# OneWalkman/EDGE-YOLO

Measured on AMD Instinct MI355X. Metric: images/sec @ 640x640 fp16 (EdgeLine-YOLO detection forward path: backbone + DWT neck + GFLv2 head decode + batched NMS), higher is better.
Workload: dtype f16; 1 GPU; yolo11n-test.yaml (scale n, nc=80) predict path, 640x640, batch 32/GPU, conf 0.25 iou 0.7 max_det 300, random-init weights, default head biases (DENSE NMS regime: mean detections/img 300); regime=dense, global_batch=32, imgsz=640, nc=80

## Files before the change

### edge-yolo_amd/_lib.py

```python
import ctypes as C
import os

import torch

_HERE = os.path.dirname(os.path.abspath(__file__))
LIB_PATH = os.path.join(_HERE, "csrc", "libedgeyolo_hip.so")

F16, F32 = 0, 1
ACT_NONE, ACT_SILU, ACT_RELU, ACT_SIGMOID = 0, 1, 2, 3
ATTN_AREA_F32, ATTN_AREA_F16, ATTN_AREA_MFMA = 401, 402, 403
ATTN_FLASH_MFMA, ATTN_FLASH_F32, ATTN_FLASH_F16 = 500, 501, 502
DWG_PLAIN, DWG_GATE, DWG_RESIDUAL = 0, 1, 2
MASK_GT_STACK, MASK_GT_INDEX = 0, 1


class HipLibraryError(RuntimeError):
    pass


class ConvDesc(C.Structure):
    _fields_ = [
        ("dtype", C.c_int32), ("B", C.c_int32), ("H", C.c_int32), ("W", C.c_int32), ("Ho", C.c_int32), ("Wo", C.c_int32),
        ("Cout", C.c_int32), ("k", C.c_int32), ("stride", C.c_int32), ("pad", C.c_int32), ("act", C.c_int32), ("nsrc", C.c_int32),
        ("src", C.c_void_p * 2), ("src_C", C.c_int32 * 2), ("src_cstride", C.c_int32 * 2), ("src_up", C.c_int32 * 2),
        ("w", C.c_void_p), ("bias", C.c_void_p), ("y", C.c_void_p), ("y_cstride", C.c_int32),
        ("res", C.c_void_p), ("res_cstride", C.c_int32), ("out_scale", C.c_float),
        ("addz", C.c_void_p), ("addz_cstride", C.c_int32), ("addz_H", C.c_int32), ("addz_W", C.c_int32), ("ngroup", C.c_int32),
        ("src_gstride", C.c_int64), ("y_gstride", C.c_int64), ("w_gstride", C.c_int64), ("w_gmax", C.c_int32),
    ]


class ConvDirectDesc(C.Structure):
    _fields_ = [
        ("dtype", C.c_int32), ("B", C.c_int32), ("H", C.c_int32), ("W", C.c_int32), ("Cin", C.c_int32), ("Ho", C.c_int32),
        ("Wo", C.c_int32), ("Cout", C.c_int32), ("k", C.c_int32), ("stride", C.c_int32), ("pad", C.c_int32), ("groups", C.c_int32),
        ("act", C.c_int32), ("x", C.c_void_p), ("x_cstride", C.c_int32), ("w_oihw", C.c_void_p), ("bias", C.c_void_p),
        ("y", C.c_void_p), ("y_cstride", C.c_int32),
    ]


class BlockStage(C.Structure):
    _fields_ = [
        ("op", C.c_int32), ("H", C.c_int32), ("W", C.c_int32), ("Ho", C.c_int32), ("Wo", C.c_int32),
        ("k", C.c_int32), ("stride", C.c_int32), ("act", C.c_int32), ("nsrc", C.c_int32),
        ("src", C.c_int64 * 2), ("src_ext", C.c_int32 * 2), ("src_img", C.c_int64 * 2), ("src_cs", C.c_int32 * 2), ("src_C", C.c_int32 * 2),
        ("w", C.c_void_p), ("bias", C.c_void_p), ("w_g", C.c_int64), ("w_gmax", C.c_int32),
        ("y", C.c_int64), ("y_ext", C.c_int32), ("y_img", C.c_int64), ("y_cs", C.c_int32), ("Cout", C.c_int32),
        ("has_res", C.c_int32), ("res", C.c_int64), ("res_ext", C.c_int32), ("res_img", C.c_int64), ("res_cs", C.c_int32),
        ("has_addz", C.c_int32), ("addz", C.c_int64), ("addz_ext", C.c_int32), ("addz_img", C.c_int64), ("addz_cs", C.c_int32), ("addz_H", C.c_int32),
        ("addz_W", C.c_int32), ("out_scale", C.c_float),
        ("ngroup", C.c_int32), ("src_g", C.c_int64), ("y_g", C.c_int64), ("heads", C.c_int32),
        ("kpad", C.c_int32), ("nt_pack", C.c_int32), ("mt", C.c_int32), ("nti", C.c_int32), ("lds", C.c_int32), ("tile_nti", C.c_int32), ("tile_src_lds", C.c_int32 * 2), ("tile_src_lcs", C.c_int32 * 2), ("tile_y_lds", C.c_int32), ("tile_y_lcs", C.c_int32), ("tile_res_lds", C.c_int32), ("tile_res_lcs", C.c_int32), ("tile_lds_bytes", C.c_int32), ("zsy", C.c_float), ("zsx", C.c_float),
    ]
# ... 16 lines not shown
    "ey_conv_pack_nt": (_i, [_i]),
    "ey_conv_chain_klen": (_i, [_i]),
    "ey_conv_chain_kperm": (_i, [_i, _vp, _i]),
    "ey_conv_pw_chain": (_i, [_i, _i, _i, _i, _i, _i, _i, _vp, _i, _vp, _vp, _i, _vp, _vp, _i, _vp, _i, _vp]),
    "ey_conv2d_direct": (_i, [C.POINTER(ConvDirectDesc), _vp]),
    "ey_stem_conv": (_i, [_i, _i, _i, _i, _i, _i, _i, _i, _vp, _vp, _vp, _vp, _i, _vp]),
    "ey_dwconv": (_i, [_i, _i, _i, _i, _i, _i, _i, _vp, _i, _vp, _vp, _vp, _i, _vp]),
    "ey_dsconv": (_i, [_i, _i, _i, _i, _i, _i, _i, _i, _vp, _i, _vp, _vp, _i, _vp, _vp, _vp, _i, _vp, _i, _vp]),
    "ey_dsconv_toeplitz_bytes": (_sz, [_i, _i]),
    "ey_dsconv_pack_toeplitz": (_i, [_i, _i, _vp, _vp, _sz]),
    "ey_dsconv_tz": (_i, [_i, _i, _i, _i, _i, _i, _i, _i, _vp, _i, _vp, _vp, _vp, _i, _vp, _vp, _vp, _i, _vp, _i, _vp]),
    "ey_dsconv_last_variant": (_i, []),
    "ey_conv_pw_conv3s2": (_i, [_i, _i, _i, _i, _vp, _i, _i, _vp, _i, _i, _i, _vp, _vp, _i, _i, _vp, _vp, _i, _vp, _i, _vp]),
    "ey_stem_pair": (_i, [_i, _i, _i, _vp, _vp, _vp, _i, _i, _vp, _vp, _i, _vp, _i, _vp]),
    "ey_dsb_pair": (_i, [_i, _i, _i, _i, _i, _i, _i, _i, _vp, _i, _vp, _vp, _vp, _vp, _vp, _vp, _i, _vp, _i, _vp]),
    "ey_dwt_haar": (_i, [_i, _i, _i, _i, _i, _vp, _i, _vp, _i, _vp]),
    "ey_dwt": (_i, [_i, _i, _i, _i, _i, _i, _vp, _vp, _i, _vp, _i, _vp]),
    "ey_wavelet_z": (_i, [_i, _i, _i, _i, _i, _vp, _i, _vp, C.c_long, _vp, _vp, _vp, _i, _vp]),
    "ey_wavelet_z2": (_i, [_i, _i, _i, _i, _i, _i, _vp, _i, _vp, _vp, _i, _vp, C.c_long, _vp, _vp, _vp, _i, _vp]),
    "ey_sppf_pool": (_i, [_i, _i, _i, _i, _i, _vp, _i, _vp, _vp, _vp, _i, _vp]),
    "ey_copy_nhwc": (_i, [_i, _i, _i, _i, _i, _i, _vp, _i, _vp, _i, _vp]),
    "ey_scale_add_channels": (_i, [_i, _i, _i, _i, _i, _vp, _i, _vp, _vp, _i, _vp, _i, _vp]),
    "ey_avgpool2": (_i, [_i, _i, _i, _i, _i, _vp, _i, _vp, _i, _vp]),
    "ey_dwconv_s2": (_i, [_i, _i, _i, _i, _i, _i, _i, _vp, _i, _vp, _vp, _vp, _i, _vp]),
    "ey_hypergraph_workspace_bytes": (_sz, [_i, _i, _i, _i]),
    "ey_hypergraph_conv": (_i, [_i, _i, _i, _i, _i, _i, _i, _vp, _i, _vp, _i, _vp, _vp, _vp, _vp, _vp, _vp, _vp, _vp, _vp, _vp, _sz, _vp]),
    "ey_nchw_to_nhwc": (_i, [_i, _i, _i, _i, _i, _vp, _vp, _i, _vp]),
    "ey_nhwc_to_nchw": (_i, [_i, _i, _i, _i, _i, _vp, _i, _vp, _vp]),
    "ey_letterbox": (_i, [_i, _vp, _i, _i, _i, _vp, _i, _i, _i, _i, _i, _i, _i, _i, _vp]),
    "ey_copy_linear": (_i, [_vp, _vp, _sz, _vp]),
# ... 145 lines not shown
```

### edge-yolo_amd/csrc/api.cpp

```cpp
#include <stdarg.h>
#include <stdio.h>
#include <stddef.h>
#include <string.h>
#include "../../include/edgeyolo_hip.h"
#include "tune.h"

static thread_local char g_err[512] = "";

int ey_set_error(int code, const char* fmt, ...) {
  va_list ap;
  va_start(ap, fmt);
  vsnprintf(g_err, sizeof(g_err), fmt, ap);
  va_end(ap);
  return code;
}

extern "C" const char* ey_last_error(void) { return g_err; }
extern "C" int ey_version(void) { return 1; }
extern "C" size_t ey_abi_sizeof(int which) { return which == 0 ? sizeof(ey_conv_desc) : which == 1 ? sizeof(ey_conv_direct_desc) : 0; }

EyTune g_ey_tune;
#define EY_T(f) {#f, offsetof(EyTune, f)}
static const struct { const char* name; size_t off; } k_tunables[] = {
    EY_T(tiles_per_wave), EY_T(mt2_min_m), EY_T(small_m), EY_T(small_wmb), EY_T(halo_min_c), EY_T(ws_lds_kb), EY_T(ws_wg_cu), EY_T(ws_k3_minnt), EY_T(tile_wlds),
    EY_T(tile_s2_minc), EY_T(tile_s2_minm), EY_T(grid_div), EY_T(c3r), EY_T(tile_minwg), EY_T(tile_flat), EY_T(tile_mink), EY_T(pwr_m), EY_T(pwr_frags), EY_T(pw_m),
    EY_T(pw_waves), EY_T(pw_wmb), EY_T(ds_p), EY_T(tz_kmask), EY_T(tz_minpx), EY_T(ds_strip), EY_T(stem_mfma), EY_T(linattn_mfma), EY_T(softattn_mfma), EY_T(areaattn_mfma), EY_T(c3p), EY_T(c3p_min_m), EY_T(c3p_fast), EY_T(c3s), EY_T(c3s_mt4_m), EY_T(c3s_min_work), EY_T(c3s_cfg), EY_T(nms_fast_k), EY_T(nms_mask_wg), EY_T(sppf_min_wg), EY_T(sppf_cv), EY_T(dsb_pair), EY_T(dsb_max_px), EY_T(dsb_rb), EY_T(dsb_fixed), EY_T(dsb_p2), EY_T(stem_pair), EY_T(pw3), EY_T(pw3_min_px), EY_T(pw3_skew), EY_T(pwn), EY_T(pwn_max_m), EY_T(pwn_ntw), EY_T(pwc), EY_T(xcd_map), EY_T(nms_mask_k), EY_T(head_lean), EY_T(head_fuse)};
static long* tunable(const char* name) {
  if (!name) return nullptr;
  for (const auto& t : k_tunables)
    if (!strcmp(t.name, name)) return (long*)((char*)&g_ey_tune + t.off);
  return nullptr;
}
extern "C" int ey_tune_set(const char* name, long value) {
  long* p = tunable(name);
  if (!p) return ey_set_error(EY_EINVAL, "ey_tune_set: unknown tunable '%s'", name ? name : "(null)");
  *p = value;
  return EY_OK;
}
extern "C" long ey_tune_get(const char* name) {
  const long* p = tunable(name);
  return p ? *p : -1;
// ... 2 lines not shown
```

### edge-yolo_amd/csrc/dsb.hip

```cpp
#include "common.h"
#include "tune.h"

struct DsbP {
  int B, H, W, act, add;
  const void* x; int xCs; unsigned xBytes;
  const void* wdw1; const void* wpw1; const float* b1;
  const void* wdw2; const void* wpw2; const float* b2;
  void* y; int yCs;
  int RB, Kpad;
};

#define DSB_SLACK 8

template <int K, int KS, int P, bool LAST>
__device__ __forceinline__ void dsb_stage(const DsbP& p, int b, const f16* s_src, int srcW, int src_row0, const f16* s_w, const void* wpw, const float* bias_g,
                                          int row_lo, int row_hi, f16* s_dst, int dstW, int dst_row0, int dst_pad, const f16* s_res, int resW, int res_row0,
                                          int res_pad) {
  constexpr int C = 32 * KS, NT = 2 * KS, CP = C + 8, NX = P + K - 1;
  const int lane = threadIdx.x & 63, r = lane & 15, g = lane >> 4, wave = threadIdx.x >> 6, nwave = blockDim.x >> 6;
  const int ch0 = g * 4 * NT;
  Vec8<f16> af[KS][NT];
  {
    const __amdgpu_buffer_rsrc_t rw = ey_rsrc(wpw, (unsigned)(16 * NT * p.Kpad * (int)sizeof(f16)));
    const unsigned wvoff = (unsigned)((r * p.Kpad + 8 * g) * (int)sizeof(f16));
#pragma unroll
    for (int ks = 0; ks < KS; ++ks)
#pragma unroll
      for (int nt = 0; nt < NT; ++nt) BufLoad8<f16>::load(af[ks][nt], rw, wvoff, (nt * 16 * p.Kpad + ks * 32) * (int)sizeof(f16));
  }
  float bias[4 * NT];
#pragma unroll
  for (int i = 0; i < 4 * NT; ++i) bias[i] = bias_g ? bias_g[ch0 + i] : 0.f;
  const int WS = (p.W + P - 1) / P;
  const int nstrip = (row_hi - row_lo) * WS;
  for (int unit = wave; unit * 16 < nstrip; unit += nwave) {
    const int si = unit * 16 + r;
    const bool sv = si < nstrip;
    const int sic = sv ? si : nstrip - 1;
    const int ry = sic / WS, x0 = (sic - ry * WS) * P, oy = row_lo + ry;
    Vec8<f16> bf[KS][P];
#pragma unroll
    for (int ks = 0; ks < KS; ++ks) {
      const int cb = ks * 32 + 8 * g;
      float acc[P][8];
#pragma unroll
      for (int q = 0; q < P; ++q)
#pragma unroll
        for (int i = 0; i < 8; ++i) acc[q][i] = 0.f;
      const f16* base = s_src + ((oy - K / 2 - src_row0) * srcW + x0) * CP + cb;
#pragma unroll
      for (int ky = 0; ky < K; ++ky) {
        Vec8<f16> xr[NX];
#pragma unroll
        for (int j = 0; j < NX; ++j) xr[j].load(base + (ky * srcW + j) * CP);
#pragma unroll
        for (int kx = 0; kx < K; ++kx) {
          Vec8<f16> w;
          w.load(s_w + (ky * K + kx) * C + cb);
#pragma unroll
          for (int q = 0; q < P; ++q) ey_fma8_mix(xr[q + kx], w, acc[q]);
        }
      }
#pragma unroll
      for (int q = 0; q < P; ++q)
#pragma unroll
        for (int i = 0; i < 8; ++i) bf[ks][q].set(i, acc[q][i]);
    }
#pragma unroll
    for (int q = 0; q < P; ++q) {
      f32x4 pacc[NT];
#pragma unroll
      for (int nt = 0; nt < NT; ++nt) pacc[nt] = (f32x4)0.f;
#pragma unroll
      for (int ks = 0; ks < KS; ++ks)
#pragma unroll
        for (int nt = 0; nt < NT; ++nt) pacc[nt] = __builtin_amdgcn_mfma_f32_16x16x32_f16(af[ks][nt].v, bf[ks][q].v, pacc[nt], 0, 0, 0);
      const int ox = x0 + q;
      if (!sv || ox >= p.W) continue;
      float v[4 * NT];
#pragma unroll
      for (int nt = 0; nt < NT; ++nt)
// ... 19 lines not shown
            Vec8<f16> rr;
            rr.load(rp + 8 * h);
#pragma unroll
            for (int j = 0; j < 8; ++j) v[8 * h + j] += rr.get(j);
          }
          Vec8<f16> o;
#pragma unroll
          for (int j = 0; j < 8; ++j) o.set(j, v[8 * h + j]);
          o.store(yp + 8 * h);
        }
      }
    }
  }
}

template <int K1, int K2, int KS, int P1, int P2>
__global__ __launch_bounds__(512) void dsb_pair_kernel(DsbP p) {
  extern __shared__ __attribute__((aligned(16))) char smem[];
  constexpr int C = 32 * KS, CP = C + 8, CV = C / 8, R1 = K1 / 2, R2 = K2 / 2, PPI = 512 / CV;
  const int RI = p.RB + 2 * (R1 + R2), WI = p.W + 2 * R1, RM = p.RB + 2 * R2, WM = p.W + 2 * R2;
  f16* s_in = reinterpret_cast<f16*>(smem);
  f16* s_mid = s_in + (RI * WI + DSB_SLACK) * CP;
  f16* s_w1 = s_mid + (RM * WM + DSB_SLACK) * CP;
  f16* s_w2 = s_w1 + K1 * K1 * C;
  const int tid = threadIdx.x, b = blockIdx.y, y0 = blockIdx.x * p.RB;
  {
    const __amdgpu_buffer_rsrc_t rx = ey_rsrc(p.x, p.xBytes);
    const int cv = tid % CV, NP = RI * WI, iy0 = y0 - R1 - R2;
    constexpr int U = 4;
    int base = tid / CV;
    bool first = true;
    do {
// ... 19 lines not shown
          w.load((const f16*)p.wdw2 + v * 8);
          w.store(s_w2 + v * 8);
        }
      }
#pragma unroll
      for (int j = 0; j < U; ++j) {
        const int px = base + j * PPI;
        if (px < NP) t[j].store(s_in + px * CP + cv * 8);
      }
      base += U * PPI;
    } while (base < NP);
  }
  __syncthreads();
  {
    const int lo = y0 - R2 < 0 ? 0 : y0 - R2, hi = y0 + p.RB + R2 > p.H ? p.H : y0 + p.RB + R2;
    dsb_stage<K1, KS, P1, false>(p, b, s_in, WI, y0 - R1 - R2, s_w1, p.wpw1, p.b1, lo, hi, s_mid, WM, y0 - R2, R2, nullptr, 0, 0, 0);
  }
  __syncthreads();
  {
    const int hi = y0 + p.RB > p.H ? p.H : y0 + p.RB;
    dsb_stage<K2, KS, P2, true>(p, b, s_mid, WM, y0 - R2, s_w2, p.wpw2, p.b2, y0, hi, nullptr, 0, 0, 0, s_in, WI, y0 - R1 - R2, R1);
  }
}

static size_t dsb_lds_bytes(int W, int C, int k1, int k2, int RB) {
  const int CP = C + 8, r1 = k1 / 2, r2 = k2 / 2;
  return ((size_t)((RB + 2 * (r1 + r2)) * (W + 2 * r1) + DSB_SLACK) + (size_t)((RB + 2 * r2) * (W + 2 * r2) + DSB_SLACK)) * CP * 2 + (size_t)(k1 * k1 + k2 * k2) * C * 2;
}

static int dsb_band_rows(int B, int H, int W, int C, int k1, int k2) {
  static int ncu = 0;
  if (!ncu) {
    int dev = 0;
    hipDeviceProp_t prop;
    if (hipGetDevice(&dev) == hipSuccess && hipGetDeviceProperties(&prop, dev) == hipSuccess) ncu = prop.multiProcessorCount;
    if (ncu < 1) ncu = 256;
  }
// ... 49 lines not shown
  const int bands = (H + RB - 1) / RB;
  const size_t lds = dsb_lds_bytes(W, C, k1, k2, RB);
  hipStream_t st = (hipStream_t)stream;
  int P2 = (int)tune().dsb_p2;
  if (P2 != 1 && P2 != 2 && P2 != 4) P2 = RB * ((W + 1) / 2) < 64 ? 1 : 2;
#define DSB(KV, KSV)                                                          \
  if (k2 == KV && C == 32 * KSV) {                                            \
    if (P2 == 1) return dsb_launch<3, KV, KSV, 2, 1>(p, bands, lds, st);      \
    if (P2 == 4) return dsb_launch<3, KV, KSV, 2, 4>(p, bands, lds, st);      \
    return dsb_launch<3, KV, KSV, 2, 2>(p, bands, lds, st);                   \
  }
  DSB(5, 1) DSB(7, 1) DSB(5, 2) DSB(7, 2)
#undef DSB
  return ey_set_error(EY_EINVAL, "dsb_pair: k2=%d C=%d", k2, C);
}
```

### edge-yolo_amd/csrc/tune.h

```cpp
#pragma once
struct EyTune {
  long tiles_per_wave = 0;
  long mt2_min_m = 300000;
  long small_m = 100000;
  long small_wmb = 48;
  long halo_min_c = 48;
  long ws_lds_kb = 76;
  long ws_wg_cu = 2;
  long ws_k3_minnt = 0;
  long tile_wlds = 1;
  long tile_s2_minc = 64;
  long tile_s2_minm = 40000;
  long grid_div = 1;
  long c3p = 1;
  long c3p_min_m = 40000;
  long c3p_fast = 1;
  long c3s = 1;
  long c3s_mt4_m = 100000;
  long c3s_min_work = 20000;
  long c3s_cfg = 0;
  long c3r = 1;
  long tile_minwg = 400;
  long tile_flat = 1;
  long tile_mink = 0;
// ... 4 lines not shown
  long pw_wmb = 64;
  long xcd_map = 31;
  long pwc = 1;
  long pwn = 1;
  long pwn_max_m = 110000;
  long pwn_ntw = 0;
  long ds_p = 0;
  long tz_kmask = 168;
  long tz_minpx = 100000;
  long ds_strip = 1;
  long dsb_pair = 1;
  long dsb_max_px = 300000;
  long dsb_rb = 0;
  long dsb_p2 = 0;
  long dsb_fixed = 100;
  long stem_pair = 1;
  long pw3 = 1;
  long pw3_skew = 8;
  long pw3_min_px = 100000;
  long stem_mfma = 1;
  long linattn_mfma = 1;
  long softattn_mfma = 1;
  long areaattn_mfma = 1;
  long sppf_min_wg = 128;
  long sppf_cv = 0;
  long nms_mask_wg = 0;
  long nms_mask_k = 1536;
  long head_fuse = 2;
  long head_lean = 1;
  long nms_fast_k = 2048;
// ... 4 lines not shown
```

### edge-yolo_amd/nn/_ops.py

```python
import ctypes

import torch

from .. import _lib as L

TRACE = None
RECORD = None


def _no_block(what):
    if RECORD is not None:
        from ._block import BlockUnsupported
        raise BlockUnsupported(what)


class _NoTrace:
    def __enter__(self):
        return None

    def __exit__(self, *a):
        return False


_NT = _NoTrace()
# ... 448 lines not shown
        cs = L.cstride(x)
        if L.cstride(out) != cs or abs(((x.data_ptr() - base) // 2) % cs - ((out.data_ptr() - base) // 2) % cs) < c:
            return None
    wk1, _, wp1, b1, _, _ = _dsconv_pack(cv1, x, cv1._dw_folded, cv1._pw_folded, k1)
    wk2, _, wp2, b2, _, _ = _dsconv_pack(cv2, x, cv2._dw_folded, cv2._pw_folded, k2)
    try:
        with _tr(f"dsb_pair_kernel<{k1},{k2}>", _nb(x, out), 2.0 * B * H * W * c * (k1 * k1 + k2 * k2 + 2 * c), note=f"C{c} {H}x{W}{' +res' if add else ''}"):
            L.check(L.lib().ey_dsb_pair(L.dtype_code(x.dtype), B, H, W, c, k1, k2, L.ACT_SILU, x.data_ptr(), L.cstride(x), wk1.data_ptr(), wp1.data_ptr(),
                                        b1.data_ptr() if b1 is not None else None, wk2.data_ptr(), wp2.data_ptr(), b2.data_ptr() if b2 is not None else None,
                                        1 if add else 0, out.data_ptr(), L.cstride(out), L.stream()), "ey_dsb_pair")
    except NotImplementedError:
        return None
    return out


def dsconv(mod, x, dw_fn, pw_fn, k, act, out=None, res=None, dw_act=0):
    L.require_device(x, "dsconv")
    x = L.as_nhwc(x)
    B, c, H, W = x.shape
    es = x.element_size()
    if c % 8 or c > 256 or (L.cstride(x) * es) % 16 or x.data_ptr() % 16:
        return None

    wk, dwb, wp, bias, cout, tz = _dsconv_pack(mod, x, dw_fn, pw_fn, k)
    if out is None:
        out = L.empty_nhwc(B, cout, H, W, x.dtype, x.device)
    elif not L.is_nhwc_view(out) or tuple(out.shape) != (B, cout, H, W):
        raise ValueError("dsconv: out= must be an NHWC view of the output shape")
    if res is not None:
        res = L.as_nhwc(res)
# ... 786 lines not shown
```

### edge-yolo_amd/nn/modules/block.py

```python
import math

import torch
import torch.nn as nn
import torch.nn.functional as F

from .conv import Conv, DSConv, _Packed, fold_bn
from .. import _ops as ops
from ... import _lib as L

__all__ = ("DFL", "Proto", "SPPF", "C2f", "C3", "C3k", "C3k2", "Bottleneck", "Attention", "PSABlock", "C2PSA", "LinearAttention",
           "PSABlock_LinearAttention", "C2PSA_LinearAttention", "AAttn", "ABlock", "A2C2f", "DSBottleneck", "DSC3k", "DSC3K2_Wavelet",
           "DSC3K2", "Mlp", "CMlp", "LocalAgg", "GlobalSparseAttn", "SelfAttn", "LGLBlock", "_DSUnit", "_LGLAdapter", "_DSUnitWithLGL", "DSC3K2_LGL",
           "AdaHyperedgeGen", "AdaHGConv", "AdaHGComputation", "C3AH", "FuseModule", "HyperACE", "DownsampleConv", "FullPAD_Tunnel")


def _slot(buf, i, c):
    return buf[:, i * c:(i + 1) * c]


class _Chains(nn.Module):

    pw_chains = ("proj_ffn_cv2",)

    def _chain(self, name):
# ... 546 lines not shown
            self.m = nn.ModuleList(DSC3k(self.c, self.c, n=2, shortcut=shortcut, g=g) for _ in range(n))
        else:
            self.m = nn.ModuleList(DSBottleneck(self.c, self.c, shortcut=shortcut, e=1.0, k1=k1, k2=k2, d2=d2) for _ in range(n))
        self.wave = _WaveletEnhancer(self.c, use_ds=use_ds, wave=wave, mode=mode)

    def forward(self, x, out=None, tail=None):
        B, _, H, W = x.shape
        c, n = self.c, len(self.m)
        t = self.cv1(x)
        buf = L.empty_nhwc(B, (1 + n) * c, H, W, x.dtype, x.device)
        pre = None
        if n and isinstance(self.m[0], C3):
            _, pre = self.wave(t[:, c:], out=_slot(buf, 0, c), then=dict(mod=self.m[0], folded_fn=self.m[0]._cv12, act=L.ACT_SILU, tag="cv12"))
        else:
            self.wave(t[:, c:], out=_slot(buf, 0, c))
        for i, m in enumerate(self.m):
            if i == 0 and pre is not None:
                m(_slot(buf, i, c), out=_slot(buf, 1 + i, c), cv12=pre)
            else:
                m(_slot(buf, i, c), out=_slot(buf, 1 + i, c))
        if tail is not None:
            y = ops.pw_conv3s2(self.cv2, tail, [t[:, :c], buf])
            return y if y is not None else tail(ops.conv2d(self.cv2, [t[:, :c], buf], self.cv2.folded, 1, 1, 0, L.ACT_SILU))
        return ops.conv2d(self.cv2, [t[:, :c], buf], self.cv2.folded, 1, 1, 0, L.ACT_SILU, out=out)


class DSC3K2(C2f):

    def __init__(self, c1, c2, n=1, dsc3k=False, e=0.5, g=1, shortcut=True, k1=3, k2=7, d2=1):
        super().__init__(c1, c2, n, shortcut, g, e)
# ... 386 lines not shown
```

### include/edgeyolo_hip.h

```cpp
#ifndef EDGEYOLO_HIP_H
#define EDGEYOLO_HIP_H
#include <stddef.h>
#include <stdint.h>

#ifdef __cplusplus
extern "C" {
#endif

typedef void* ey_stream_t;

enum { EY_F16 = 0, EY_F32 = 1 };
enum { EY_ACT_NONE = 0, EY_ACT_SILU = 1, EY_ACT_RELU = 2, EY_ACT_SIGMOID = 3 };
enum { EY_OK = 0, EY_EINVAL = -1, EY_EUNSUPPORTED = -2, EY_ELAUNCH = -3 };

const char* ey_last_error(void);
int ey_version(void);
size_t ey_abi_sizeof(int which);
int ey_tune_set(const char* name, long value);
long ey_tune_get(const char* name);

typedef struct {
  int32_t dtype;
  int32_t B, H, W;
  int32_t Ho, Wo;
// ... 58 lines not shown
              const float* bias, void* y, int y_cstride, ey_stream_t stream);

int ey_dsconv(int dtype, int B, int H, int W, int Cin, int Cout, int k, int act, const void* x, int x_cstride,
              const void* w_dw_kkc, const float* dw_bias, int dw_act, const void* w_pw_packed, const float* bias, void* y, int y_cstride, const void* res,
              int res_cstride, ey_stream_t stream);

size_t ey_dsconv_toeplitz_bytes(int C, int k);
int ey_dsconv_pack_toeplitz(int C, int k, const float* w_dw_kkc_host, void* out_host, size_t out_bytes);
int ey_dsconv_tz(int dtype, int B, int H, int W, int Cin, int Cout, int k, int act, const void* x, int x_cstride,
                 const void* w_dw_kkc, const void* w_dw_toeplitz, const float* dw_bias, int dw_act, const void* w_pw_packed, const float* bias,
                 void* y, int y_cstride, const void* res, int res_cstride, ey_stream_t stream);

int ey_dsb_pair(int dtype, int B, int H, int W, int C, int k1, int k2, int act, const void* x, int x_cstride, const void* w_dw1_kkc,
                const void* w_pw1_packed, const float* bias1, const void* w_dw2_kkc, const void* w_pw2_packed, const float* bias2, int add_residual,
                void* y, int y_cstride, ey_stream_t stream);

int ey_dsconv_last_variant(void);

int ey_dwt_haar(int dtype, int B, int H, int W, int C, const void* x, int x_cstride, void* y, int y_cstride,
                ey_stream_t stream);

int ey_dwt(int dtype, int B, int H, int W, int C, int k, const float* taps, const void* x, int x_cstride, void* y, int y_cstride,
           ey_stream_t stream);

int ey_wavelet_z(int dtype, int B, int H, int W, int C, const void* x, int x_cstride, const void* w_sub_packed, long w_set_stride, const float* b_sub,
                 const void* w_z_packed, void* z, int z_cstride, ey_stream_t stream);
int ey_wavelet_z2(int dtype, int B, int H, int W, int C, int k, const float* taps, int use_ds, const void* w_dw_kkc, const void* x, int x_cstride,
                  const void* w_sub_packed, long w_set_stride, const float* b_sub, const void* w_z_packed, void* z, int z_cstride, ey_stream_t stream);

int ey_sppf_pool(int dtype, int B, int H, int W, int C, const void* x, int x_cstride, void* y1, void* y2, void* y3,
// ... 165 lines not shown
```

Baseline: 28730 images/s.

## Fuse C3k2 cv2 pointwise conv into the DSBottleneck pair kernel

Adds a dsb_pair_pw kernel path that runs the two depthwise-separable bottleneck stages and then applies the block's final 1x1 conv (cv2) over the concatenated segments (global slice, pair input, pair output) in registers via MFMA. For n==1 DSBottleneck blocks it writes the cv2 output directly, so the pair output and the concat no longer make a global-memory round trip and a separate pointwise launch is avoided. In exchange the kernel carries more registers and extra weight loads inside the last stage, which may lower occupancy. The tunable dsb_cv2 defaults to 1, which limits the path to C==32.

```diff
diff --git a/edge-yolo_amd/_lib.py b/edge-yolo_amd/_lib.py
--- a/edge-yolo_amd/_lib.py
+++ b/edge-yolo_amd/_lib.py
@@ -37,6 +37,13 @@
         ("act", C.c_int32), ("x", C.c_void_p), ("x_cstride", C.c_int32), ("w_oihw", C.c_void_p), ("bias", C.c_void_p),
         ("y", C.c_void_p), ("y_cstride", C.c_int32),
     ]
+
+
+class KSeg(C.Structure):
+    _fields_ = [("kind", C.c_int32), ("ptr", C.c_void_p), ("cstride", C.c_int32), ("C", C.c_int32)]
+
+
+KSEG_GLOBAL, KSEG_PAIR_IN, KSEG_PAIR_OUT = 0, 1, 2
 
 
 class BlockStage(C.Structure):
@@ -83,6 +90,7 @@
     "ey_conv_pw_conv3s2": (_i, [_i, _i, _i, _i, _vp, _i, _i, _vp, _i, _i, _i, _vp, _vp, _i, _i, _vp, _vp, _i, _vp, _i, _vp]),
     "ey_stem_pair": (_i, [_i, _i, _i, _vp, _vp, _vp, _i, _i, _vp, _vp, _i, _vp, _i, _vp]),
     "ey_dsb_pair": (_i, [_i, _i, _i, _i, _i, _i, _i, _i, _vp, _i, _vp, _vp, _vp, _vp, _vp, _vp, _i, _vp, _i, _vp]),
+    "ey_dsb_pair_pw": (_i, [_i, _i, _i, _i, _i, _i, _i, _i, _vp, _i, _vp, _vp, _vp, _vp, _vp, _vp, _i, _vp, _i, C.POINTER(KSeg), _i, _vp, _vp, _i, _i, _vp, _i, _vp]),
     "ey_dwt_haar": (_i, [_i, _i, _i, _i, _i, _vp, _i, _vp, _i, _vp]),
     "ey_dwt": (_i, [_i, _i, _i, _i, _i, _i, _vp, _vp, _i, _vp, _i, _vp]),
     "ey_wavelet_z": (_i, [_i, _i, _i, _i, _i, _vp, _i, _vp, C.c_long, _vp, _vp, _vp, _i, _vp]),
diff --git a/edge-yolo_amd/csrc/api.cpp b/edge-yolo_amd/csrc/api.cpp
--- a/edge-yolo_amd/csrc/api.cpp
+++ b/edge-yolo_amd/csrc/api.cpp
@@ -24,7 +24,7 @@
 static const struct { const char* name; size_t off; } k_tunables[] = {
     EY_T(tiles_per_wave), EY_T(mt2_min_m), EY_T(small_m), EY_T(small_wmb), EY_T(halo_min_c), EY_T(ws_lds_kb), EY_T(ws_wg_cu), EY_T(ws_k3_minnt), EY_T(tile_wlds),
     EY_T(tile_s2_minc), EY_T(tile_s2_minm), EY_T(grid_div), EY_T(c3r), EY_T(tile_minwg), EY_T(tile_flat), EY_T(tile_mink), EY_T(pwr_m), EY_T(pwr_frags), EY_T(pw_m),
-    EY_T(pw_waves), EY_T(pw_wmb), EY_T(ds_p), EY_T(tz_kmask), EY_T(tz_minpx), EY_T(ds_strip), EY_T(stem_mfma), EY_T(linattn_mfma), EY_T(softattn_mfma), EY_T(areaattn_mfma), EY_T(c3p), EY_T(c3p_min_m), EY_T(c3p_fast), EY_T(c3s), EY_T(c3s_mt4_m), EY_T(c3s_min_work), EY_T(c3s_cfg), EY_T(nms_fast_k), EY_T(nms_mask_wg), EY_T(sppf_min_wg), EY_T(sppf_cv), EY_T(dsb_pair), EY_T(dsb_max_px), EY_T(dsb_rb), EY_T(dsb_fixed), EY_T(dsb_p2), EY_T(stem_pair), EY_T(pw3), EY_T(pw3_min_px), EY_T(pw3_skew), EY_T(pwn), EY_T(pwn_max_m), EY_T(pwn_ntw), EY_T(pwc), EY_T(xcd_map), EY_T(nms_mask_k), EY_T(head_lean), EY_T(head_fuse)};
+    EY_T(pw_waves), EY_T(pw_wmb), EY_T(ds_p), EY_T(tz_kmask), EY_T(tz_minpx), EY_T(ds_strip), EY_T(stem_mfma), EY_T(linattn_mfma), EY_T(softattn_mfma), EY_T(areaattn_mfma), EY_T(c3p), EY_T(c3p_min_m), EY_T(c3p_fast), EY_T(c3s), EY_T(c3s_mt4_m), EY_T(c3s_min_work), EY_T(c3s_cfg), EY_T(nms_fast_k), EY_T(nms_mask_wg), EY_T(sppf_min_wg), EY_T(sppf_cv), EY_T(dsb_pair), EY_T(dsb_max_px), EY_T(dsb_rb), EY_T(dsb_fixed), EY_T(dsb_p2), EY_T(dsb_cv2), EY_T(stem_pair), EY_T(pw3), EY_T(pw3_min_px), EY_T(pw3_skew), EY_T(pwn), EY_T(pwn_max_m), EY_T(pwn_ntw), EY_T(pwc), EY_T(xcd_map), EY_T(nms_mask_k), EY_T(head_lean), EY_T(head_fuse)};
 static long* tunable(const char* name) {
   if (!name) return nullptr;
   for (const auto& t : k_tunables)
diff --git a/edge-yolo_amd/csrc/dsb.hip b/edge-yolo_amd/csrc/dsb.hip
--- a/edge-yolo_amd/csrc/dsb.hip
+++ b/edge-yolo_amd/csrc/dsb.hip
@@ -10,10 +10,173 @@
   int RB, Kpad;
 };
 
+struct DsbPwP {
+  int nseg, kind[3];
+  const void* g; int gCs; unsigned gBytes;
+  const void* w; const float* bias;
+  int act, Cout, Kpad;
+  void* out; int outCs;
+};
+
 #define DSB_SLACK 8
 
-template <int K, int KS, int P, bool LAST>
-__device__ __forceinline__ void dsb_stage(const DsbP& p, int b, const f16* s_src, int srcW, int src_row0, const f16* s_w, const void* wpw, const float* bias_g,
+template <int KS, int P, int NTC>
+__device__ __forceinline__ void dsb_pw_tail(const DsbP& p, const DsbPwP& c, int b, const Vec8<f16> (&af)[KS][2 * KS], const Vec8<f16> (&bf)[KS][P],
+                                            const float (&bias)[8 * KS], const Vec8<f16> (&gf)[KS][P], const Vec8<f16> (&cf)[3][KS == 1 ? NTC : 1],
+                                            __amdgpu_buffer_rsrc_t rw2, unsigned wvoff2, bool sv, int x0, int oy, const f16* s_res, int resW, int res_row0,
+                                            int res_pad) {
+  constexpr int C = 32 * KS, NT = 2 * KS, CP = C + 8, QG = (KS == 1 || P < 2) ? 1 : 2, NS = 3 * KS;
+  const int lane = threadIdx.x & 63, g = lane >> 4;
+  const int ch0 = g * 4 * NT, chc = g * 4 * NTC;
+  const __amdgpu_buffer_rsrc_t rb2 = ey_rsrc(c.bias, c.bias ? (unsigned)(c.Cout * (int)sizeof(float)) : 0u);
+  if constexpr (KS > 1) asm volatile("" : "+v"(wvoff2));
+  Vec8<f16> xf[KS][P], of[KS][P];
+#pragma unroll
+  for (int q = 0; q < P; ++q) {
+    f32x4 pacc[NT];
+#pragma unroll
+    for (int nt = 0; nt < NT; ++nt) pacc[nt] = (f32x4)0.f;
+#pragma unroll
+    for (int ks = 0; ks < KS; ++ks)
+#pragma unroll
+      for (int nt = 0; nt < NT; ++nt) pacc[nt] = __builtin_amdgcn_mfma_f32_16x16x32_f16(af[ks][nt].v, bf[ks][q].v, pacc[nt], 0, 0, 0);
+    const int ox = x0 + q;
+    const bool ok = sv && ox < p.W;
+    float v[4 * NT];
+#pragma unroll
+    for (int nt = 0; nt < NT; ++nt)
+#pragma unroll
+      for (int j = 0; j < 4; ++j) v[4 * nt + j] = pacc[nt][j] + bias[4 * nt + j];
+    ey_act_n(v, p.act);
+    f16* px = const_cast<f16*>(s_res) + ((oy - res_row0) * resW + ox + res_pad) * CP;
+    if constexpr (KS > 1) {
+#pragma unroll
+      for (int ks = 0; ks < KS; ++ks) xf[ks][q].load(px + ks * 32 + 8 * g);
+    }
+    Vec8<f16> o[NT / 2];
+#pragma unroll
+    for (int h = 0; h < NT / 2; ++h) {
+      Vec8<f16> rr;
+      rr.load(px + ch0 + 8 * h);
+      if (p.add) {
+#pragma unroll
+        for (int j = 0; j < 8; ++j) v[8 * h + j] += rr.get(j);
+      }
+#pragma unroll
+      for (int j = 0; j < 8; ++j) o[h].set(j, v[8 * h + j]);
+      if constexpr (KS == 1) xf[0][q] = rr;
+    }
+    if (p.y && ok) {
+      f16* yp = (f16*)p.y + (((long)b * p.H + oy) * p.W + ox) * p.yCs + ch0;
+#pragma unroll
+      for (int h = 0; h < NT / 2; ++h) o[h].store(yp + 8 * h);
+    }
+    if constexpr (KS == 1) {
+      of[0][q] = o[0];
+    } else {
+      __builtin_amdgcn_fence(__ATOMIC_RELEASE, "wavefront");
+      __builtin_amdgcn_wave_barrier();
+      if (ok) {
+#pragma unroll
+        for (int h = 0; h < NT / 2; ++h) o[h].store(px + ch0 + 8 * h);
+      }
+      __builtin_amdgcn_fence(__ATOMIC_RELEASE, "wavefront");
+      __builtin_amdgcn_wave_barrier();
+      __builtin_amdgcn_fence(__ATOMIC_ACQUIRE, "wavefront");
+#pragma unroll
+      for (int ks = 0; ks < KS; ++ks) of[ks][q].load(px + ks * 32 + 8 * g);
+    }
+  }
+  unsigned mk[3][3];
+#pragma unroll
+  for (int sg = 0; sg < 3; ++sg)
+#pragma unroll
+    for (int k = 0; k < 3; ++k) mk[sg][k] = c.kind[sg] == k ? 0xffffffffu : 0u;
+  auto frag = [&](int s, int q) -> f16x8 {
+    const int sg = s / KS, ks = s % KS;
+    const ey_u32x4 a = __builtin_bit_cast(ey_u32x4, gf[ks][q].v), x = __builtin_bit_cast(ey_u32x4, xf[ks][q].v), o = __builtin_bit_cast(ey_u32x4, of[ks][q].v);
+    return __builtin_bit_cast(f16x8, (a & (ey_u32x4)mk[sg][EY_KSEG_GLOBAL]) | (x & (ey_u32x4)mk[sg][EY_KSEG_PAIR_IN]) | (o & (ey_u32x4)mk[sg][EY_KSEG_PAIR_OUT]));
+  };
+  constexpr int NH = (KS > 1 && NTC == 8) ? 2 : 1, NTH = NTC / NH;
+#pragma unroll
+  for (int q0 = 0; q0 < P; q0 += QG) {
+#pragma unroll
+    for (int hf = 0; hf < NH; ++hf) {
+      f32x4 acc[QG][NTH];
+#pragma unroll
+      for (int qq = 0; qq < QG; ++qq)
+#pragma unroll
+        for (int nt = 0; nt < NTH; ++nt) acc[qq][nt] = (f32x4)0.f;
+      if constexpr (KS == 1) {
+#pragma unroll
+        for (int s = 0; s < NS; ++s) {
+          if (s >= c.nseg) break;
+#pragma unroll
+          for (int qq = 0; qq < QG; ++qq) {
+            const f16x8 bq = frag(s, q0 + qq);
+#pragma unroll
+            for (int nt = 0; nt < NTH; ++nt) acc[qq][nt] = __builtin_amdgcn_mfma_f32_16x16x32_f16(cf[s][nt].v, bq, acc[qq][nt], 0, 0, 0);
+          }
+        }
+      } else {
+        Vec8<f16> wq[2][NTH];
+        auto issue = [&](int s, Vec8<f16> (&w)[NTH]) {
+#pragma unroll
+          for (int nt = 0; nt < NTH; ++nt)
+            BufLoad8<f16>::load(w[nt], rw2, s / KS < c.nseg ? wvoff2 : EY_OOB, ((hf * NTH + nt) * 16 * c.Kpad + s * 32) * (int)sizeof(f16));
+        };
+        issue(0, wq[0]);
+#pragma unroll
+        for (int s = 0; s < NS; ++s) {
+          if (s + 1 < NS) issue(s + 1, wq[(s + 1) & 1]);
+          __builtin_amdgcn_sched_barrier(0);
+          if (s / KS < c.nseg) {
+#pragma unroll
+            for (int qq = 0; qq < QG; ++qq) {
+              const f16x8 bq = frag(s, q0 + qq);
+#pragma unroll
+              for (int nt = 0; nt < NTH; ++nt) acc[qq][nt] = __builtin_amdgcn_mfma_f32_16x16x32_f16(wq[s & 1][nt].v, bq, acc[qq][nt], 0, 0, 0);
+            }
+          }
+          __builtin_amdgcn_sched_barrier(0);
+        }
+      }
+      const int chh = chc + 4 * NTH * hf;
+#pragma unroll
+      for (int qq = 0; qq < QG; ++qq) {
+        const int ox = x0 + q0 + qq;
+        if (sv && ox < p.W) {
+          float v[4 * NTH];
+#pragma unroll
+          for (int nt = 0; nt < NTH; ++nt) {
+            const f32x4 bq = __builtin_bit_cast(f32x4, __builtin_amdgcn_raw_buffer_load_b128(rb2, (chh + 4 * nt) * (int)sizeof(float), 0, 0));
+#pragma unroll
+            for (int j = 0; j < 4; ++j) v[4 * nt + j] = acc[qq][nt][j] + bq[j];
+          }
+          if (c.act == EY_ACT_SILU) {
+#pragma unroll
+            for (int i = 0; i < 4 * NTH; ++i) v[i] = ey_silu_rn(v[i]);
+          } else {
+            ey_act_n(v, c.act);
+          }
+          f16* op = (f16*)c.out + (((long)b * p.H + oy) * p.W + ox) * c.outCs + chh;
+#pragma unroll
+          for (int h = 0; h < NTH / 2; ++h) {
+            if (chh + 8 * h + 8 <= c.Cout) {
+              Vec8<f16> o;
+#pragma unroll
+              for (int j = 0; j < 8; ++j) o.set(j, v[8 * h + j]);
+              o.store(op + 8 * h);
+            }
+          }
+        }
+      }
+    }
+  }
+}
+
+template <int K, int KS, int P, bool LAST, int NTC = 0>
+__device__ __forceinline__ void dsb_stage(const DsbP& p, const DsbPwP& c, int b, const f16* s_src, int srcW, int src_row0, const f16* s_w, const void* wpw, const float* bias_g,
                                           int row_lo, int row_hi, f16* s_dst, int dstW, int dst_row0, int dst_pad, const f16* s_res, int resW, int res_row0,
                                           int res_pad) {
   constexpr int C = 32 * KS, NT = 2 * KS, CP = C + 8, NX = P + K - 1;
@@ -31,6 +194,18 @@
   float bias[4 * NT];
 #pragma unroll
   for (int i = 0; i < 4 * NT; ++i) bias[i] = bias_g ? bias_g[ch0 + i] : 0.f;
+  constexpr bool PW = LAST && NTC > 0, PWREG = PW && KS == 1;
+  constexpr int NTR = PWREG ? NTC : 1, PG = PW ? P : 1;
+  Vec8<f16> cf[3][NTR];
+  const __amdgpu_buffer_rsrc_t rw2 = ey_rsrc(PW ? c.w : nullptr, PW ? (unsigned)(16 * NTC * c.Kpad * (int)sizeof(f16)) : 0u);
+  const __amdgpu_buffer_rsrc_t rg = ey_rsrc(PW ? c.g : nullptr, PW ? c.gBytes : 0u);
+  const unsigned wvoff2 = PW ? (unsigned)((r * c.Kpad + 8 * g) * (int)sizeof(f16)) : 0u;
+  if constexpr (PWREG) {
+#pragma unroll
+    for (int s = 0; s < 3; ++s)
+#pragma unroll
+      for (int nt = 0; nt < NTC; ++nt) BufLoad8<f16>::load(cf[s][nt], rw2, s < c.nseg ? wvoff2 : EY_OOB, (nt * 16 * c.Kpad + s * 32) * (int)sizeof(f16));
+  }
   const int WS = (p.W + P - 1) / P;
   const int nstrip = (row_hi - row_lo) * WS;
   for (int unit = wave; unit * 16 < nstrip; unit += nwave) {
@@ -38,6 +213,16 @@
     const bool sv = si < nstrip;
     const int sic = sv ? si : nstrip - 1;
     const int ry = sic / WS, x0 = (sic - ry * WS) * P, oy = row_lo + ry;
+    Vec8<f16> gf[KS][PG];
+    if constexpr (PW) {
+#pragma unroll
+      for (int q = 0; q < P; ++q) {
+        const bool ok = c.g && sv && x0 + q < p.W;
+        const unsigned off = ok ? (unsigned)(((((b * p.H + oy) * p.W + x0 + q) * c.gCs) + 8 * g) * (int)sizeof(f16)) : EY_OOB;
+#pragma unroll
+        for (int ks = 0; ks < KS; ++ks) BufLoad8<f16>::load(gf[ks][q], rg, off, ks * 32 * (int)sizeof(f16));
+      }
+    }
     Vec8<f16> bf[KS][P];
 #pragma unroll
     for (int ks = 0; ks < KS; ++ks) {
@@ -65,6 +250,10 @@
       for (int q = 0; q < P; ++q)
 #pragma unroll
         for (int i = 0; i < 8; ++i) bf[ks][q].set(i, acc[q][i]);
+    }
+    if constexpr (PW) {
+      dsb_pw_tail<KS, P, NTC>(p, c, b, af, bf, bias, gf, cf, rw2, wvoff2, sv, x0, oy, s_res, resW, res_row0, res_pad);
+      continue;
     }
 #pragma unroll
     for (int q = 0; q < P; ++q) {
@@ -114,8 +303,8 @@
   }
 }
 
-template <int K1, int K2, int KS, int P1, int P2>
-__global__ __launch_bounds__(512) void dsb_pair_kernel(DsbP p) {
+template <int K1, int K2, int KS, int P1, int P2, int NTC>
+__device__ __forceinline__ void dsb_pair_body(const DsbP& p, const DsbPwP& c) {
   extern __shared__ __attribute__((aligned(16))) char smem[];
   constexpr int C = 32 * KS, CP = C + 8, CV = C / 8, R1 = K1 / 2, R2 = K2 / 2, PPI = 512 / CV;
   const int RI = p.RB + 2 * (R1 + R2), WI = p.W + 2 * R1, RM = p.RB + 2 * R2, WM = p.W + 2 * R2;
@@ -165,13 +354,23 @@
   __syncthreads();
   {
     const int lo = y0 - R2 < 0 ? 0 : y0 - R2, hi = y0 + p.RB + R2 > p.H ? p.H : y0 + p.RB + R2;
-    dsb_stage<K1, KS, P1, false>(p, b, s_in, WI, y0 - R1 - R2, s_w1, p.wpw1, p.b1, lo, hi, s_mid, WM, y0 - R2, R2, nullptr, 0, 0, 0);
+    dsb_stage<K1, KS, P1, false>(p, c, b, s_in, WI, y0 - R1 - R2, s_w1, p.wpw1, p.b1, lo, hi, s_mid, WM, y0 - R2, R2, nullptr, 0, 0, 0);
   }
   __syncthreads();
   {
     const int hi = y0 + p.RB > p.H ? p.H : y0 + p.RB;
-    dsb_stage<K2, KS, P2, true>(p, b, s_mid, WM, y0 - R2, s_w2, p.wpw2, p.b2, y0, hi, nullptr, 0, 0, 0, s_in, WI, y0 - R1 - R2, R1);
-  }
+    dsb_stage<K2, KS, P2, true, NTC>(p, c, b, s_mid, WM, y0 - R2, s_w2, p.wpw2, p.b2, y0, hi, nullptr, 0, 0, 0, s_in, WI, y0 - R1 - R2, R1);
+  }
+}
+
+template <int K1, int K2, int KS, int P1, int P2>
+__global__ __launch_bounds__(512) void dsb_pair_kernel(DsbP p) {
+  dsb_pair_body<K1, K2, KS, P1, P2, 0>(p, DsbPwP{});
+}
+
+template <int K2, int KS, int P2, int NTC>
+__global__ __launch_bounds__(512) void dsb_pair_pw_kernel(DsbP p, DsbPwP c) {
+  dsb_pair_body<3, K2, KS, 2, P2, NTC>(p, c);
 }
 
 static size_t dsb_lds_bytes(int W, int C, int k1, int k2, int RB) {
@@ -251,3 +450,84 @@
 #undef DSB
   return ey_set_error(EY_EINVAL, "dsb_pair: k2=%d C=%d", k2, C);
 }
+
+template <int K2, int KS, int P2, int NTC>
+static int dsb_pw_launch(const DsbP& p, const DsbPwP& c, int bands, size_t lds, hipStream_t st) {
+  static size_t reserved = 0;
+  if (lds > 64 * 1024 && lds > reserved) {
+    if (hipFuncSetAttribute((const void*)dsb_pair_pw_kernel<K2, KS, P2, NTC>, hipFuncAttributeMaxDynamicSharedMemorySize, (int)lds) != hipSuccess)
+      return ey_set_error(EY_ELAUNCH, "dsb_pair_pw: cannot reserve %zu B of LDS", lds);
+    reserved = lds;
+  }
+  hipLaunchKernelGGL((dsb_pair_pw_kernel<K2, KS, P2, NTC>), dim3((unsigned)bands, (unsigned)p.B), dim3(512), lds, st, p, c);
+  EY_LAUNCH_CHECK("ey_dsb_pair_pw");
+  return EY_OK;
+}
+
+static bool dsb_ranges_overlap(const void* a, long abytes, const void* b, long bbytes) {
+  const uintptr_t a0 = (uintptr_t)a, b0 = (uintptr_t)b;
+  return a0 < b0 + (uintptr_t)bbytes && b0 < a0 + (uintptr_t)abytes;
+}
+
+extern "C" int ey_dsb_pair_pw(int dtype, int B, int H, int W, int C, int k1, int k2, int act, const void* x, int x_cstride, const void* w_dw1_kkc,
+                              const void* w_pw1_packed, const float* bias1, const void* w_dw2_kkc, const void* w_pw2_packed, const float* bias2,
+                              int add_residual, void* y, int y_cstride, const ey_kseg* segs, int nseg, const void* w_pw_packed, const float* bias_pw, int act_pw,
+                              int Cout, void* out, int out_cstride, ey_stream_t stream) {
+  EY_CHECK(x && out && w_dw1_kkc && w_pw1_packed && w_dw2_kkc && w_pw2_packed && w_pw_packed && segs, "dsb_pair_pw: null pointer");
+  EY_CHECK(B > 0 && H > 0 && W > 0 && Cout > 0, "dsb_pair_pw: bad extent");
+  EY_CHECK(x_cstride >= C && out_cstride >= Cout && (!y || y_cstride >= C), "dsb_pair_pw: cstride");
+  const int es = 2;
+  const long M = (long)B * H * W;
+  const long xbytes = ((M - 1) * x_cstride + C) * es, ybytes = y ? ((M - 1) * y_cstride + C) * es : 0, obytes = ((M - 1) * out_cstride + Cout) * es;
+  bool fits = (tune().dsb_cv2 == 3 || (tune().dsb_cv2 != 0 && C == 32)) && tune().dsb_pair && dtype == EY_F16 && (C == 32 || C == 64) && k1 == 3 && (k2 == 5 || k2 == 7) && B <= 65535 &&
+              xbytes < (1L << 31) && ybytes < (1L << 31) && obytes < (1L << 31) && (x_cstride * es) % 16 == 0 && ey_aligned(x, 16) &&
+              (!y || ((y_cstride * es) % 16 == 0 && ey_aligned(y, 16))) && (out_cstride * es) % 16 == 0 && ey_aligned(out, 16) && ey_aligned(w_dw1_kkc, 16) &&
+              ey_aligned(w_dw2_kkc, 16) && ey_aligned(w_pw1_packed, 16) && ey_aligned(w_pw2_packed, 16) && ey_aligned(w_pw_packed, 16) && M <= tune().dsb_max_px &&
+              nseg >= 1 && nseg <= 3 && Cout % 16 == 0 && Cout >= 48 && Cout <= 128 && Cout != 80;
+  fits = fits && !dsb_ranges_overlap(out, obytes, x, xbytes) && !(y && dsb_ranges_overlap(out, obytes, y, ybytes));
+  DsbPwP c;
+  c.nseg = nseg; c.g = nullptr; c.gCs = 0; c.gBytes = 0;
+  for (int s = 0; s < 3; ++s) c.kind[s] = EY_KSEG_PAIR_IN;
+  for (int s = 0; fits && s < nseg; ++s) {
+    const ey_kseg& sg = segs[s];
+    c.kind[s] = sg.kind;
+    if (sg.kind == EY_KSEG_GLOBAL) {
+      const long gbytes = ((M - 1) * sg.cstride + C) * es;
+      fits = !c.g && sg.ptr && sg.C == C && sg.cstride >= C && (sg.cstride * es) % 16 == 0 && ey_aligned(sg.ptr, 16) && gbytes < (1L << 31) &&
+             !dsb_ranges_overlap(out, obytes, sg.ptr, gbytes);
+      c.g = sg.ptr; c.gCs = sg.cstride; c.gBytes = (unsigned)gbytes;
+    } else if (sg.kind == EY_KSEG_PAIR_IN || sg.kind == EY_KSEG_PAIR_OUT) {
+      fits = sg.C == C;
+    } else {
+      fits = false;
+    }
+  }
+  if (!fits)
+    return ey_set_error(EY_EUNSUPPORTED, "dsb_pair_pw: outside the fused kernel (f16, C 32/64, k 3 -> 5/7, small maps, 1-3 segments of C channels with one global view at "
+                                         "most, Cout 48/64/96/112/128, 16-byte aligned views, output apart from the inputs) or not selected by tunable dsb_cv2");
+  const int RB = dsb_band_rows(B, H, W, C, k1, k2);
+  if (RB < 1) return ey_set_error(EY_EUNSUPPORTED, "dsb_pair_pw: a one-row band of a %d-wide map does not fit LDS", W);
+  DsbP p;
+  p.B = B; p.H = H; p.W = W; p.act = act; p.add = add_residual;
+  p.x = x; p.xCs = x_cstride; p.xBytes = (unsigned)xbytes;
+  p.wdw1 = w_dw1_kkc; p.wpw1 = w_pw1_packed; p.b1 = bias1; p.wdw2 = w_dw2_kkc; p.wpw2 = w_pw2_packed; p.b2 = bias2;
+  p.y = y; p.yCs = y_cstride;
+  p.RB = RB; p.Kpad = ey_conv_kpad(C, es);
+  c.w = w_pw_packed; c.bias = bias_pw; c.act = act_pw; c.Cout = Cout; c.Kpad = ey_conv_kpad(nseg * C, es);
+  c.out = out; c.outCs = out_cstride;
+  const int bands = (H + RB - 1) / RB;
+  const size_t lds = dsb_lds_bytes(W, C, k1, k2, RB);
+  hipStream_t st = (hipStream_t)stream;
+  int P2 = (int)tune().dsb_p2;
+  if (P2 != 1 && P2 != 2 && P2 != 4) P2 = RB * ((W + 1) / 2) < 64 ? 1 : 2;
+  const int ntc = Cout <= 64 ? 4 : 8;
+#define DSBPW(KV, KSV, NTCV)                                                         \
+  if (k2 == KV && C == 32 * KSV && ntc == NTCV) {                                    \
+    if (P2 == 1) return dsb_pw_launch<KV, KSV, 1, NTCV>(p, c, bands, lds, st);       \
+    if (P2 == 4) return dsb_pw_launch<KV, KSV, 4, NTCV>(p, c, bands, lds, st);       \
+    return dsb_pw_launch<KV, KSV, 2, NTCV>(p, c, bands, lds, st);                    \
+  }
+  DSBPW(5, 1, 4) DSBPW(7, 1, 4) DSBPW(5, 2, 4) DSBPW(7, 2, 4) DSBPW(5, 1, 8) DSBPW(7, 1, 8) DSBPW(5, 2, 8) DSBPW(7, 2, 8)
+#undef DSBPW
+  return ey_set_error(EY_EINVAL, "dsb_pair_pw: k2=%d C=%d Cout=%d", k2, C, Cout);
+}
diff --git a/edge-yolo_amd/csrc/tune.h b/edge-yolo_amd/csrc/tune.h
--- a/edge-yolo_amd/csrc/tune.h
+++ b/edge-yolo_amd/csrc/tune.h
@@ -42,6 +42,7 @@
   long dsb_rb = 0;
   long dsb_p2 = 0;
   long dsb_fixed = 100;
+  long dsb_cv2 = 1;
   long stem_pair = 1;
   long pw3 = 1;
   long pw3_skew = 8;
diff --git a/edge-yolo_amd/nn/_ops.py b/edge-yolo_amd/nn/_ops.py
--- a/edge-yolo_amd/nn/_ops.py
+++ b/edge-yolo_amd/nn/_ops.py
@@ -486,6 +486,54 @@
     return out
 
 
+def dsb_pair_pw(cv1, cv2, x, add, pw, a, out=None, y=None):
+    L.require_device(x, "dsb_pair_pw")
+    if RECORD is not None or x.dtype != torch.float16 or isinstance(a, VirtualCat) or a.dtype != x.dtype or L.lib().ey_tune_get(b"dsb_cv2") == 0:
+        return None
+    x, a = L.as_nhwc(x), L.as_nhwc(a)
+    B, c, H, W = x.shape
+    k1, k2 = cv1.dw.kernel_size[0], cv2.dw.kernel_size[0]
+    pc = pw.conv
+    from .modules.conv import _act_code
+    if (c not in (32, 64) or k1 != 3 or k2 not in (5, 7) or cv1.pw.out_channels != c or cv2.pw.out_channels != c or cv2.dw.in_channels != c
+            or any(m.dw.stride != (1, 1) or m.dw.dilation != (1, 1) or m.dw.padding != (m.dw.kernel_size[0] // 2,) * 2 or m.dw.bias is not None for m in (cv1, cv2))
+            or tuple(a.shape) != (B, c, H, W) or pc.kernel_size != (1, 1) or pc.stride != (1, 1) or pc.groups != 1 or pc.in_channels != 3 * c
+            or pc.out_channels % 16 or pc.out_channels > 128):
+        return None
+    cout = pc.out_channels
+    if out is None:
+        out = L.empty_nhwc(B, cout, H, W, x.dtype, x.device)
+    elif not L.is_nhwc_view(out) or tuple(out.shape) != (B, cout, H, W) or out.dtype != x.dtype:
+        raise ValueError("dsb_pair_pw: out= must be an NHWC view of the output shape")
+    if y is not None:
+        if not L.is_nhwc_view(y) or tuple(y.shape) != (B, c, H, W) or y.dtype != x.dtype:
+            raise ValueError("dsb_pair_pw: y= must be an NHWC view of the pair's shape")
+        base = x.untyped_storage().data_ptr()
+        if y.untyped_storage().data_ptr() == base:
+            cs = L.cstride(x)
+            if L.cstride(y) != cs or abs(((x.data_ptr() - base) // 2) % cs - ((y.data_ptr() - base) // 2) % cs) < c:
+                return None
+    wk1, _, wp1, b1, _, _ = _dsconv_pack(cv1, x, cv1._dw_folded, cv1._pw_folded, k1)
+    wk2, _, wp2, b2, _, _ = _dsconv_pack(cv2, x, cv2._dw_folded, cv2._pw_folded, k2)
+    wp, bp = _conv_pack(pw, x, 3 * c, 1)[:2]
+    segs = (L.KSeg * 3)()
+    segs[0].kind, segs[0].ptr, segs[0].cstride, segs[0].C = L.KSEG_GLOBAL, a.data_ptr(), L.cstride(a), c
+    segs[1].kind, segs[1].C = L.KSEG_PAIR_IN, c
+    segs[2].kind, segs[2].C = L.KSEG_PAIR_OUT, c
+    M = B * H * W
+    try:
+        with _tr(f"dsbcv2_kernel<{k1},{k2}>", _nb(x, a, out, y), 2.0 * M * c * (k1 * k1 + k2 * k2 + 2 * c) + 2.0 * M * 3 * c * cout,
+                 note=f"C{c} {H}x{W}{' +res' if add else ''} -> {3 * c}->{cout} k1"):
+            L.check(L.lib().ey_dsb_pair_pw(L.dtype_code(x.dtype), B, H, W, c, k1, k2, L.ACT_SILU, x.data_ptr(), L.cstride(x), wk1.data_ptr(), wp1.data_ptr(),
+                                           b1.data_ptr() if b1 is not None else None, wk2.data_ptr(), wp2.data_ptr(), b2.data_ptr() if b2 is not None else None,
+                                           1 if add else 0, y.data_ptr() if y is not None else None, L.cstride(y) if y is not None else 0, segs, 3, wp.data_ptr(),
+                                           bp.data_ptr() if bp is not None else None, _act_code(pw.act), cout, out.data_ptr(), L.cstride(out), L.stream()),
+                    "ey_dsb_pair_pw")
+    except NotImplementedError:
+        return None
+    return out
+
+
 def dsconv(mod, x, dw_fn, pw_fn, k, act, out=None, res=None, dw_act=0):
     L.require_device(x, "dsconv")
     x = L.as_nhwc(x)
diff --git a/edge-yolo_amd/nn/modules/block.py b/edge-yolo_amd/nn/modules/block.py
--- a/edge-yolo_amd/nn/modules/block.py
+++ b/edge-yolo_amd/nn/modules/block.py
@@ -584,6 +584,11 @@
             _, pre = self.wave(t[:, c:], out=_slot(buf, 0, c), then=dict(mod=self.m[0], folded_fn=self.m[0]._cv12, act=L.ACT_SILU, tag="cv12"))
         else:
             self.wave(t[:, c:], out=_slot(buf, 0, c))
+        if n == 1 and isinstance(self.m[0], DSBottleneck):
+            m = self.m[0]
+            y = ops.dsb_pair_pw(m.cv1, m.cv2, _slot(buf, 0, c), m.add, self.cv2, t[:, :c], out=out if tail is None else None)
+            if y is not None:
+                return y if tail is None else tail(y)
         for i, m in enumerate(self.m):
             if i == 0 and pre is not None:
                 m(_slot(buf, i, c), out=_slot(buf, 1 + i, c), cv12=pre)
diff --git a/include/edgeyolo_hip.h b/include/edgeyolo_hip.h
--- a/include/edgeyolo_hip.h
+++ b/include/edgeyolo_hip.h
@@ -96,6 +96,20 @@
 int ey_dsb_pair(int dtype, int B, int H, int W, int C, int k1, int k2, int act, const void* x, int x_cstride, const void* w_dw1_kkc,
                 const void* w_pw1_packed, const float* bias1, const void* w_dw2_kkc, const void* w_pw2_packed, const float* bias2, int add_residual,
                 void* y, int y_cstride, ey_stream_t stream);
+
+#define EY_KSEG_GLOBAL 0
+#define EY_KSEG_PAIR_IN 1
+#define EY_KSEG_PAIR_OUT 2
+typedef struct ey_kseg {
+  int kind;
+  const void* ptr;
+  int cstride;
+  int C;
+} ey_kseg;
+int ey_dsb_pair_pw(int dtype, int B, int H, int W, int C, int k1, int k2, int act, const void* x, int x_cstride, const void* w_dw1_kkc,
+                   const void* w_pw1_packed, const float* bias1, const void* w_dw2_kkc, const void* w_pw2_packed, const float* bias2, int add_residual,
+                   void* y, int y_cstride, const ey_kseg* segs, int nseg, const void* w_pw_packed, const float* bias_pw, int act_pw, int Cout, void* out,
+                   int out_cstride, ey_stream_t stream);
 
 int ey_dsconv_last_variant(void);
 
```

After: 28750 images/s (median of 3 runs). About the same (+0.1%).
